# ShuhangGu/DASR

Measured on AMD Instinct MI355X. Metric: SR train images/sec (4x, 128->512), higher is better.
Workload: dtype bf16 MFMA operands, fp32 accumulate / fp32 residual stream

## Files before the change

dasr_amd/csrc/common.h:

```cpp
#pragma once
#include <hip/hip_runtime.h>
#include <hip/hip_ext.h>
#include <stdint.h>
#include "../../include/dasr_hip.h"

typedef __bf16 bf16_t;
typedef __attribute__((ext_vector_type(8))) __bf16 bf16x8;
typedef __attribute__((ext_vector_type(4))) __bf16 bf16x4;
typedef __attribute__((ext_vector_type(4))) short s16x4;
typedef _Float16 f16_t;
typedef __attribute__((ext_vector_type(8))) _Float16 f16x8;
typedef __attribute__((ext_vector_type(4))) _Float16 f16x4;
typedef __attribute__((ext_vector_type(16))) float f32x16;
typedef __attribute__((ext_vector_type(4))) float f32x4;
typedef __attribute__((ext_vector_type(4))) unsigned int u32x4;
typedef __attribute__((ext_vector_type(2))) unsigned int u32x2;

#define DASR_LDS __attribute__((address_space(3)))

#define HIP_TRY(expr)                                   \
    do {                                                \
        hipError_t _e = (expr);                         \
        if (_e != hipSuccess) return (int)_e;           \
    } while (0)

__device__ __forceinline__ float bf16_to_f32(bf16_t v) { return (float)v; }

__device__ __forceinline__ bf16_t f32_to_bf16(float v) { return (bf16_t)v; }

__device__ __forceinline__ void split_bf16(float v, bf16_t& hi, bf16_t& lo) {
    hi = (bf16_t)v;
    lo = (bf16_t)(v - (float)hi);
}

__device__ __forceinline__ void split_f16(float v, bf16_t& hi, bf16_t& lo) {
    const f16_t h = (f16_t)v;
    hi = __builtin_bit_cast(bf16_t, h);
    lo = __builtin_bit_cast(bf16_t, (f16_t)(v - (float)h));
}

template <bool F16>
__device__ __forceinline__ f32x16 mfma16(bf16x8 a, bf16x8 b, f32x16 c) {
    if constexpr (F16) return __builtin_amdgcn_mfma_f32_32x32x16_f16(__builtin_bit_cast(f16x8, a), __builtin_bit_cast(f16x8, b), c, 0, 0, 0);
    else return __builtin_amdgcn_mfma_f32_32x32x16_bf16(a, b, c, 0, 0, 0);
}

__device__ __forceinline__ float wave_sum(float v) {
#pragma unroll
    for (int o = 32; o > 0; o >>= 1) v += __shfl_xor(v, o, 64);
    return v;
}

static inline hipStream_t as_stream(void* s) { return (hipStream_t)s; }

struct dasr_red {
    float* part;
    unsigned* ticket;
};
dasr_red dasr_red_scratch(const void* key_acc, hipStream_t s, unsigned nblocks, int k);
int dasr_red_error();

template <int K>
__device__ __forceinline__ void grid_sum_commit(const dasr_red r, const float (&v)[K], float* const (&acc)[K], const float (&coef)[K]) {
    if (!r.part) return;
    __shared__ unsigned gs_last;
    __shared__ float gs_red[K][4];
    const unsigned nb = gridDim.x;
    if (threadIdx.x == 0) {
#pragma unroll
        for (int k = 0; k < K; ++k) __hip_atomic_store(r.part + (size_t)k * nb + blockIdx.x, v[k], __ATOMIC_RELAXED, __HIP_MEMORY_SCOPE_AGENT);
        asm volatile("s_waitcnt vmcnt(0)" ::: "memory");
        gs_last = __hip_atomic_fetch_add(r.ticket, 1u, __ATOMIC_RELAXED, __HIP_MEMORY_SCOPE_AGENT) == nb - 1u;
    }
    __syncthreads();
    if (!gs_last) return;
#pragma unroll
    for (int k = 0; k < K; ++k) {
        float s = 0.f;
        for (unsigned i = threadIdx.x; i < nb; i += 256u) s += __hip_atomic_load(r.part + (size_t)k * nb + i, __ATOMIC_RELAXED, __HIP_MEMORY_SCOPE_AGENT);
        s = wave_sum(s);
        if ((threadIdx.x & 63) == 0) gs_red[k][threadIdx.x >> 6] = s;
    }
    __syncthreads();
    if (threadIdx.x == 0) {
#pragma unroll
        for (int k = 0; k < K; ++k)
            if (acc[k]) atomicAdd(acc[k], ((gs_red[k][0] + gs_red[k][1]) + (gs_red[k][2] + gs_red[k][3])) * coef[k]);
        __hip_atomic_store(r.ticket, 0u, __ATOMIC_RELAXED, __HIP_MEMORY_SCOPE_AGENT);
    }
}

bool dasr_prof_slot(const char* tag, hipEvent_t* e0, hipEvent_t* e1);
#define DASR_LAUNCH_TAG(tag, kfn, grid, block, lds, s, ...)                                         \
    do {                                                                                            \
        hipEvent_t _e0 = nullptr, _e1 = nullptr;                                                    \
        if (dasr_prof_slot(tag, &_e0, &_e1)) hipExtLaunchKernelGGL(kfn, grid, block, lds, s, _e0, _e1, 0, __VA_ARGS__); \
        else hipLaunchKernelGGL(kfn, grid, block, lds, s, __VA_ARGS__);                             \
    } while (0)
#define DASR_LAUNCH(kfn, ...) DASR_LAUNCH_TAG(#kfn, kfn, __VA_ARGS__)
```

dasr_amd/csrc/misc.hip:

```cpp
#include "common.h"
#include <string.h>
#include <atomic>
#include <condition_variable>
#include <map>
#include <mutex>
#include <thread>
#include <tuple>

namespace {

__global__ void pack_kernel(const dasr_pack_desc* __restrict__ descs, int ndesc, long long total,
                            const long long* __restrict__ prefix, const float* __restrict__ params, bf16_t* __restrict__ packed) {
    const long long gid = (long long)blockIdx.x * blockDim.x + threadIdx.x;
    if (gid >= total) return;
    int lo = 0, hi = ndesc - 1;
    while (lo < hi) {
        const int mid = (lo + hi + 1) >> 1;
        if (prefix[mid] <= gid) lo = mid; else hi = mid - 1;
    }
    const dasr_pack_desc& D = descs[lo];
    long long q = gid - prefix[lo];
    const int lane = q & 63;
    q >>= 6;
    const int mi = q % D.mt;
    q /= D.mt;
    const int tap = q % D.ntaps;
    q /= D.ntaps;
    const int nchunks = D.cin_pad >> 4;
    const int ckv = q % nchunks;
    const int mg = q / nchunks;
    const int oc = (mg * D.mt + mi) * 32 + (lane & 31);
    const int kreal = D.fmt >= 3 ? nchunks / 3 : nchunks;
    const int part = ckv / kreal, ck = ckv - part * kreal;
    const int c0 = ck * 16 + 8 * (lane >> 5);
    bf16x8 vh, vl;
#pragma unroll
    for (int e = 0; e < 8; ++e) {
        const int cin = c0 + e;
        float v = 0.f;
        if (oc < D.cout) {
            for (int s = 0; s < D.nseg; ++s) {
                const dasr_pack_seg& S = D.seg[s];
                const int ci = cin - S.cin_start;
                if (ci >= 0 && ci < S.cin_len) {
                    const int st = D.tapmap[tap];
                    const unsigned msk = tap < 16 ? D.tapmask[tap] : 0u;
                    const bool okc = !S.transpose || ci < S.src_cout;
                    const long long base = !S.transpose ? S.src_off + ((long long)oc * S.src_cin + S.src_c0 + ci) * D.src_ntaps
                                                        : S.src_off + ((long long)ci * S.src_cin + S.src_c0 + oc) * D.src_ntaps;
                    if (msk && okc) {
                        float acc = 0.f;
                        for (int k = 0; k < D.src_ntaps && k < 16; ++k)
                            if (msk & (1u << k)) acc += params[base + k];
                        v = acc;
                    } else if (st >= 0 && okc) {
                        v = params[base + st];
                    }
                }
            }
        }
        bf16_t h, l;
        split_bf16(v, h, l);
        if (D.fmt == 1) h = __builtin_bit_cast(bf16_t, (f16_t)v);
        if (D.fmt == 2 || D.fmt == 3) split_f16(v, h, l);
        if (D.fmt >= 3 && part == 2) h = l;
        vh[e] = h;
        vl[e] = l;
    }
    const long long o = D.dst_off + (gid - prefix[lo]) * 8;
    *(bf16x8*)(packed + o) = vh;
    if (D.lo_off) *(bf16x8*)(packed + o + D.lo_off) = vl;
}

__global__ void nchw_to_blocked_kernel(const float* __restrict__ src, int N, int C, int H, int W, dasr_tensor df, dasr_tensor db) {
    const int ncb = (C + 15) >> 4;
    const long long total = (long long)N * ncb * H * W;
    const long long i = (long long)blockIdx.x * blockDim.x + threadIdx.x;
    if (i >= total) return;
    const int x = i % W;
    long long t = i / W;
    const int y = t % H;
    t /= H;
    const int cb = t % ncb;
    const int n = t / ncb;
    float v[16];
#pragma unroll
    for (int j = 0; j < 16; ++j) {
        const int c = cb * 16 + j;
        v[j] = c < C ? src[(((long long)n * C + c) * H + y) * W + x] : 0.f;
    }
    const size_t po = ((size_t)y * W + x) * 16;
    if (df.p) {
        float* d = (float*)df.p + (size_t)n * df.n_stride + (size_t)cb * df.cb_stride + po;
#pragma unroll
        for (int j = 0; j < 4; ++j) ((f32x4*)d)[j] = f32x4{v[4 * j], v[4 * j + 1], v[4 * j + 2], v[4 * j + 3]};
    }
    if (db.p) {
        bf16_t* d = (bf16_t*)db.p + (size_t)n * db.n_stride + (size_t)cb * db.cb_stride + po;
        bf16x8 a, b;
#pragma unroll
        for (int j = 0; j < 8; ++j) {
            a[j] = (bf16_t)v[j];
            b[j] = (bf16_t)v[8 + j];
        }
        ((bf16x8*)d)[0] = a;
        ((bf16x8*)d)[1] = b;
    }
}

__global__ void blocked_to_nchw_kernel(dasr_tensor s, int N, int C, int H, int W, float* __restrict__ dst) {
    const long long total = (long long)N * C * H * W;
    const long long i = (long long)blockIdx.x * blockDim.x + threadIdx.x;
    if (i >= total) return;
    const int x = i % W;
    long long t = i / W;
    const int y = t % H;
    t /= H;
    const int c = t % C;
    const int n = t / C;
    dst[i] = ((const float*)s.p)[(size_t)n * s.n_stride + (size_t)(c >> 4) * s.cb_stride + ((size_t)y * W + x) * 16 + (c & 15)];
}

__global__ void l1_loss_kernel(dasr_tensor sr, const float* __restrict__ hr, const float* __restrict__ wm, int N, int C, int H, int W,
                               float coef, float* loss_acc, dasr_tensor grad, int accumulate, float gscale, dasr_red rs) {
    const long long total = (long long)N * H * W;
    const long long i = (long long)blockIdx.x * blockDim.x + threadIdx.x;
    float part = 0.f;
    if (i < total) {
        const int x = i % W;
        long long t = i / W;
        const int y = t % H;
        const int n = t / H;
        const size_t po = ((size_t)y * W + x) * 16;
        const float* s = (const float*)sr.p + (size_t)n * sr.n_stride + po;
        const float wgt = wm ? wm[((long long)n * H + y) * W + x] : 1.f;
        float g[16];
#pragma unroll
        for (int j = 0; j < 16; ++j) g[j] = 0.f;
        for (int c = 0; c < C; ++c) {
            const float d = s[c] - hr[(((long long)n * C + c) * H + y) * W + x];
            if (accumulate & 2) {
                part += wgt * d * d;
                g[c] = 2.f * coef * wgt * d;
            } else {
                part += wgt * fabsf(d);
                g[c] = coef * wgt * (d > 0.f ? 1.f : (d < 0.f ? -1.f : 0.f));
            }
        }
        if (grad.p && (accumulate & 4)) {
            f16_t* gp = (f16_t*)grad.p + (size_t)n * grad.n_stride + po;
            for (int j = 0; j < (C + 3) / 4; ++j) {
                f16x4 o;
#pragma unroll
                for (int e = 0; e < 4; ++e) o[e] = (f16_t)(g[4 * j + e] * gscale);
                ((f16x4*)gp)[j] = o;
            }
        } else if (grad.p) {
            float* gp = (float*)grad.p + (size_t)n * grad.n_stride + po;
#pragma unroll
            for (int j = 0; j < 4; ++j) {
                f32x4 o = {g[4 * j], g[4 * j + 1], g[4 * j + 2], g[4 * j + 3]};
                if (accumulate & 1) o += ((const f32x4*)gp)[j];
                ((f32x4*)gp)[j] = o;
            }
        }
    }
    part = wave_sum(part);
    __shared__ float red[4];
    if ((threadIdx.x & 63) == 0) red[threadIdx.x >> 6] = part;
    __syncthreads();
    const float v[1] = {red[0] + red[1] + red[2] + red[3]};
    float* const acc[1] = {loss_acc};
    const float cf[1] = {coef};
    grid_sum_commit<1>(rs, v, acc, cf);
}

__global__ void downsum2x_kernel(dasr_tensor src, int N, int C, int H, int W, dasr_tensor mask, int mask_f32, float slope,
                                 dasr_tensor df, dasr_tensor db) {
    const int ncb = (C + 15) >> 4;
    const long long total = (long long)N * ncb * H * W * 4;
    const long long gi = (long long)blockIdx.x * blockDim.x + threadIdx.x;
    if (gi >= total) return;
    const int q = gi & 3;
    const long long i = gi >> 2;
    const int x = i % W;
    long long t = i / W;
    const int y = t % H;
    t /= H;
    const int cb = t % ncb;
    const int n = t / ncb;
    const float* s = (const float*)src.p + (size_t)n * src.n_stride + (size_t)cb * src.cb_stride + q * 4;
    const int W2 = 2 * W;
    f32x4 a = *(const f32x4*)(s + ((size_t)(2 * y) * W2 + 2 * x) * 16);
    a += *(const f32x4*)(s + ((size_t)(2 * y) * W2 + 2 * x + 1) * 16);
    a += *(const f32x4*)(s + ((size_t)(2 * y + 1) * W2 + 2 * x) * 16);
    a += *(const f32x4*)(s + ((size_t)(2 * y + 1) * W2 + 2 * x + 1) * 16);
    const size_t po = ((size_t)y * W + x) * 16 + q * 4;
    if (mask.p) {
        const size_t mo = (size_t)n * mask.n_stride + (size_t)cb * mask.cb_stride + po;
        float m[4];
        if (mask_f32) {
            const f32x4 mv = *(const f32x4*)((const float*)mask.p + mo);
            for (int j = 0; j < 4; ++j) m[j] = mv[j];
        } else {
            const bf16x4 mv = *(const bf16x4*)((const bf16_t*)mask.p + mo);
            for (int j = 0; j < 4; ++j) m[j] = (float)mv[j];
        }
        for (int j = 0; j < 4; ++j) a[j] = m[j] > 0.f ? a[j] : a[j] * slope;
    }
    if (df.p) *(f32x4*)((float*)df.p + (size_t)n * df.n_stride + (size_t)cb * df.cb_stride + po) = a;
    if (db.p) {
        bf16x4 o;
        for (int j = 0; j < 4; ++j) o[j] = (bf16_t)a[j];
        *(bf16x4*)((bf16_t*)db.p + (size_t)n * db.n_stride + (size_t)cb * db.cb_stride + po) = o;
    }
}

__global__ void axpby_kernel(dasr_tensor x, float a, dasr_tensor z, float b, int N, int C, int H, int W, dasr_tensor of,
                             dasr_tensor ob, float gamma, dasr_tensor mask, float slope, const float* slope_ptr) {
    const int ncb = (C + 15) >> 4;
    const long long per_plane = (long long)H * W * 4;
    const long long total = (long long)N * ncb * per_plane;
    const long long gi = (long long)blockIdx.x * blockDim.x + threadIdx.x;
    if (gi >= total) return;
    const long long e = (gi % per_plane) * 4;
    long long t = gi / per_plane;
    const int cb = t % ncb;
    const int n = t / ncb;
    f32x4 v = *(const f32x4*)((const float*)x.p + (size_t)n * x.n_stride + (size_t)cb * x.cb_stride + e) * a;
    if (z.p) v += *(const f32x4*)((const float*)z.p + (size_t)n * z.n_stride + (size_t)cb * z.cb_stride + e) * b;
    if (mask.p) {
        const float sl = slope_ptr ? *slope_ptr : slope;
        const f32x4 mv = *(const f32x4*)((const float*)mask.p + (size_t)n * mask.n_stride + (size_t)cb * mask.cb_stride + e);
        for (int j = 0; j < 4; ++j) v[j] = mv[j] > 0.f ? v[j] : v[j] * sl;
    }
    if (of.p) *(f32x4*)((float*)of.p + (size_t)n * of.n_stride + (size_t)cb * of.cb_stride + e) = v;
    if (ob.p) {
        bf16x4 o;
        for (int j = 0; j < 4; ++j) o[j] = (bf16_t)(v[j] * gamma);
        *(bf16x4*)((bf16_t*)ob.p + (size_t)n * ob.n_stride + (size_t)cb * ob.cb_stride + e) = o;
    }
}

__global__ void adam_kernel(float* __restrict__ p, const float* __restrict__ g, float* __restrict__ m, float* __restrict__ v,
                            long long n, float step_size, float beta1, float beta2, float eps, float wd, float inv_sqrt_bc2, int* __restrict__ nonfinite,
                            const int* __restrict__ gate) {
    if (gate && *gate != 0) return;
    bool bad = false;
    for (long long i = (long long)blockIdx.x * blockDim.x + threadIdx.x; i < n; i += (long long)gridDim.x * blockDim.x) {
        float gi = g[i];
        bad |= !(fabsf(gi) <= 3.0e38f);
        const float pi = p[i];
        if (wd != 0.f) gi += wd * pi;
        const float mi = beta1 * m[i] + (1.f - beta1) * gi;
        const float vi = beta2 * v[i] + (1.f - beta2) * gi * gi;
        m[i] = mi;
        v[i] = vi;
        const float denom = sqrtf(vi) * inv_sqrt_bc2 + eps;
        p[i] = pi - step_size * (mi / denom);
    }
    if (nonfinite && __any(bad) && (threadIdx.x & 63) == 0) atomicOr(nonfinite, 1);
}

__global__ void add_flat_kernel(float* __restrict__ y, const float* __restrict__ x, long long n) {
    for (long long i = (long long)blockIdx.x * blockDim.x + threadIdx.x; i < n; i += (long long)gridDim.x * blockDim.x) y[i] += x[i];
}

__global__ void fill_kernel(float* p, long long n, float v) {
    for (long long i = (long long)blockIdx.x * blockDim.x + threadIdx.x; i < n; i += (long long)gridDim.x * blockDim.x) p[i] = v;
}

inline unsigned blocks_for(long long total, int bs = 256) { return (unsigned)((total + bs - 1) / bs); }

}

extern "C" int dasr_pack_weights(const dasr_pack_desc* descs_dev, int32_t ndesc, int64_t total_pieces, const int64_t* piece_prefix_dev,
                                 const float* params_flat, void* packed, void* stream) {
    if (ndesc <= 0 || total_pieces <= 0) return DASR_EINVAL;
    DASR_LAUNCH(pack_kernel, dim3(blocks_for(total_pieces)), dim3(256), 0, as_stream(stream), descs_dev, ndesc,
                       (long long)total_pieces, (const long long*)piece_prefix_dev, params_flat, (bf16_t*)packed);
    return (int)hipGetLastError();
}

extern "C" int dasr_nchw_to_blocked(const float* src, int32_t N, int32_t C, int32_t H, int32_t W, dasr_tensor dst_f32,
                                    dasr_tensor dst_bf16, void* stream) {
    const long long total = (long long)N * ((C + 15) / 16) * H * W;
    if (total <= 0) return DASR_EINVAL;
    DASR_LAUNCH(nchw_to_blocked_kernel, dim3(blocks_for(total)), dim3(256), 0, as_stream(stream), src, N, C, H, W, dst_f32, dst_bf16);
    return (int)hipGetLastError();
}

extern "C" int dasr_blocked_to_nchw(dasr_tensor src, int32_t N, int32_t C, int32_t H, int32_t W, float* dst, void* stream) {
    const long long total = (long long)N * C * H * W;
    if (total <= 0) return DASR_EINVAL;
    DASR_LAUNCH(blocked_to_nchw_kernel, dim3(blocks_for(total)), dim3(256), 0, as_stream(stream), src, N, C, H, W, dst);
    return (int)hipGetLastError();
}

extern "C" int dasr_l1_loss(dasr_tensor sr, const float* hr_nchw, const float* weight_map, int32_t N, int32_t C, int32_t H, int32_t W,
                            float coef, float* loss_acc, dasr_tensor grad, int32_t accumulate, float grad_scale, void* stream) {
    const long long total = (long long)N * H * W;
    if (total <= 0 || C > 16) return DASR_EINVAL;
    if ((accumulate & 4) && (accumulate & 1)) return DASR_EINVAL;
    const dasr_red rs = dasr_red_scratch(loss_acc, as_stream(stream), blocks_for(total), 1);
    if (loss_acc && !rs.part) return dasr_red_error();
    DASR_LAUNCH(l1_loss_kernel, dim3(blocks_for(total)), dim3(256), 0, as_stream(stream), sr, hr_nchw, weight_map, N, C, H, W, coef,
                       loss_acc, grad, accumulate, grad_scale != 0.f ? grad_scale : 1.f, rs);
    return (int)hipGetLastError();
}

extern "C" int dasr_downsum2x(dasr_tensor src, int32_t N, int32_t C, int32_t H, int32_t W, dasr_tensor mask, int32_t mask_f32,
                              float slope, dasr_tensor dst_f32, dasr_tensor dst_bf16, void* stream) {
    const long long total = (long long)N * ((C + 15) / 16) * H * W * 4;
    if (total <= 0) return DASR_EINVAL;
    DASR_LAUNCH(downsum2x_kernel, dim3(blocks_for(total)), dim3(256), 0, as_stream(stream), src, N, C, H, W, mask, mask_f32, slope,
                       dst_f32, dst_bf16);
    return (int)hipGetLastError();
}

__device__ __forceinline__ float f32_rounded(float v) {
    asm("" : "+v"(v));
    return v;
}

__global__ void cvt_f16_kernel(dasr_tensor x, int N, int C, int H, int W, float scale, dasr_tensor y) {
    const int ncb = (C + 15) >> 4;
    const long long per_plane = (long long)H * W * 4, total = (long long)N * ncb * per_plane;
    const long long gi = (long long)blockIdx.x * blockDim.x + threadIdx.x;
    if (gi >= total) return;
    const long long e = (gi % per_plane) * 4;
    long long t = gi / per_plane;
    const int cb = t % ncb, n = t / ncb;
    const f32x4 v = *(const f32x4*)((const float*)x.p + (size_t)n * x.n_stride + (size_t)cb * x.cb_stride + e);
    f16x4 o;
    for (int j = 0; j < 4; ++j) o[j] = (f16_t)f32_rounded(v[j] * scale);
    *(f16x4*)((f16_t*)y.p + (size_t)n * y.n_stride + (size_t)cb * y.cb_stride + e) = o;
}

__global__ void f16_residual_kernel(dasr_tensor x, int N, int C, int H, int W, float scale, dasr_tensor y) {
    const int ncb = (C + 15) >> 4;
    const long long per_plane = (long long)H * W * 4, total = (long long)N * ncb * per_plane;
    const long long gi = (long long)blockIdx.x * blockDim.x + threadIdx.x;
    if (gi >= total) return;
    const long long e = (gi % per_plane) * 4;
    long long t = gi / per_plane;
    const int cb = t % ncb, n = t / ncb;
    const f32x4 v = *(const f32x4*)((const float*)x.p + (size_t)n * x.n_stride + (size_t)cb * x.cb_stride + e);
    const float inv = 1.f / scale;
    f32x4 o;
    for (int j = 0; j < 4; ++j) o[j] = v[j] - (float)(f16_t)f32_rounded(v[j] * scale) * inv;
    *(f32x4*)((float*)y.p + (size_t)n * y.n_stride + (size_t)cb * y.cb_stride + e) = o;
}

template <typename T>
__global__ void cvt_split16_kernel(dasr_tensor x, int N, int C, int H, int W, float scale, dasr_tensor y) {
    const int ncb = (C + 15) >> 4;
    const long long per_plane = (long long)H * W * 4, total = (long long)N * ncb * per_plane;
    const long long gi = (long long)blockIdx.x * blockDim.x + threadIdx.x;
    if (gi >= total) return;
    const long long e = (gi % per_plane) * 4;
    long long t = gi / per_plane;
    const int cb = t % ncb, n = t / ncb;
    const f32x4 v = *(const f32x4*)((const float*)x.p + (size_t)n * x.n_stride + (size_t)cb * x.cb_stride + e);
    T* yp = (T*)y.p + (size_t)n * y.n_stride + (size_t)cb * y.cb_stride + e;
    const size_t lo = (size_t)ncb * y.cb_stride;
#pragma unroll
    for (int j = 0; j < 4; ++j) {
        const float vv = f32_rounded(v[j] * scale);
        const T h = (T)vv;
        yp[j] = h;
        yp[lo + j] = (T)(vv - (float)h);
    }
}

__global__ void downsum2x_f16_kernel(dasr_tensor src, int N, int C, int H, int W, dasr_tensor mask, float slope, float out_scale, dasr_tensor df,
                                     dasr_tensor dh) {
    const int ncb = (C + 15) >> 4;
    const long long total = (long long)N * ncb * H * W * 4;
    const long long gi = (long long)blockIdx.x * blockDim.x + threadIdx.x;
    if (gi >= total) return;
    const int q = gi & 3;
    const long long i = gi >> 2;
    const int x = i % W;
    long long t = i / W;
    const int y = t % H;
    t /= H;
    const int cb = t % ncb, n = t / ncb;
    const f16_t* s = (const f16_t*)src.p + (size_t)n * src.n_stride + (size_t)cb * src.cb_stride + q * 4;
    const int W2 = 2 * W;
    float a[4] = {0.f, 0.f, 0.f, 0.f};
    for (int dy = 0; dy < 2; ++dy)
        for (int dx = 0; dx < 2; ++dx) {
            const f16x4 v = *(const f16x4*)(s + ((size_t)(2 * y + dy) * W2 + 2 * x + dx) * 16);
            for (int j = 0; j < 4; ++j) a[j] += (float)v[j];
        }
    const size_t po = ((size_t)y * W + x) * 16 + q * 4;
    if (mask.p) {
        const f16x4 mv = *(const f16x4*)((const f16_t*)mask.p + (size_t)n * mask.n_stride + (size_t)cb * mask.cb_stride + po);
        for (int j = 0; j < 4; ++j) a[j] = (float)mv[j] > 0.f ? a[j] : a[j] * slope;
    }
    for (int j = 0; j < 4; ++j) a[j] *= out_scale;
    if (df.p) *(f32x4*)((float*)df.p + (size_t)n * df.n_stride + (size_t)cb * df.cb_stride + po) = f32x4{a[0], a[1], a[2], a[3]};
    if (dh.p) {
        f16x4 o;
        for (int j = 0; j < 4; ++j) o[j] = (f16_t)a[j];
        *(f16x4*)((f16_t*)dh.p + (size_t)n * dh.n_stride + (size_t)cb * dh.cb_stride + po) = o;
    }
}

__global__ void pixel_shuffle_f16_kernel(dasr_tensor src, int N, int C4, int H, int W, dasr_tensor dst) {
    const int ncb = C4 >> 4;
    const long long total = (long long)N * ncb * H * W;
    const long long i = (long long)blockIdx.x * blockDim.x + threadIdx.x;
    if (i >= total) return;
    const int x = i % W;
    long long t = i / W;
    const int y = t % H;
    t /= H;
    const int p = t % ncb, n = t / ncb;
    const f16_t* s = (const f16_t*)src.p + (size_t)n * src.n_stride + (size_t)p * src.cb_stride + ((size_t)y * W + x) * 16;
    const f16x8 lo = *(const f16x8*)s, hi = *(const f16x8*)(s + 8);
    f16_t v[16];
    for (int j = 0; j < 8; ++j) { v[j] = lo[j]; v[8 + j] = hi[j]; }
    f16_t* d = (f16_t*)dst.p + (size_t)n * dst.n_stride + (size_t)(p >> 2) * dst.cb_stride + 4 * (p & 3);
    const int W2 = 2 * W;
    for (int k = 0; k < 4; ++k) {
        const f16x4 o = {v[k], v[4 + k], v[8 + k], v[12 + k]};
        *(f16x4*)(d + ((size_t)(2 * y + (k >> 1)) * W2 + 2 * x + (k & 1)) * 16) = o;
    }
}

__global__ void pixel_unshuffle_f16_kernel(dasr_tensor gsrc, dasr_tensor mask, float slope, int N, int C4, int H, int W, dasr_tensor gdst) {
    const int ncb = C4 >> 4;
    const long long total = (long long)N * ncb * H * W;
    const long long i = (long long)blockIdx.x * blockDim.x + threadIdx.x;
    if (i >= total) return;
    const int x = i % W;
    long long t = i / W;
    const int y = t % H;
    t /= H;
    const int p = t % ncb, n = t / ncb;
    const f16_t* g = (const f16_t*)gsrc.p + (size_t)n * gsrc.n_stride + (size_t)(p >> 2) * gsrc.cb_stride + 4 * (p & 3);
    const int W2 = 2 * W;
    f16_t v[16];
    for (int k = 0; k < 4; ++k) {
        const f16x4 q = *(const f16x4*)(g + ((size_t)(2 * y + (k >> 1)) * W2 + 2 * x + (k & 1)) * 16);
        for (int cc = 0; cc < 4; ++cc) v[4 * cc + k] = q[cc];
    }
    const size_t po = (size_t)n * gdst.n_stride + (size_t)p * gdst.cb_stride + ((size_t)y * W + x) * 16;
    if (mask.p) {
        const f16_t* m = (const f16_t*)mask.p + (size_t)n * mask.n_stride + (size_t)p * mask.cb_stride + ((size_t)y * W + x) * 16;
        for (int j = 0; j < 16; ++j) v[j] = (float)m[j] > 0.f ? v[j] : (f16_t)((float)v[j] * slope);
    }
    f16x8 lo, hi;
    for (int j = 0; j < 8; ++j) { lo[j] = v[j]; hi[j] = v[8 + j]; }
    *(f16x8*)((f16_t*)gdst.p + po) = lo;
    *(f16x8*)((f16_t*)gdst.p + po + 8) = hi;
}

extern "C" int dasr_pixel_shuffle_f16(dasr_tensor src, int32_t N, int32_t C4, int32_t H, int32_t W, dasr_tensor dst, void* stream) {
    const long long total = (long long)N * (C4 / 16) * H * W;
    if (total <= 0 || (C4 & 63) || !src.p || !dst.p) return DASR_EINVAL;
    DASR_LAUNCH(pixel_shuffle_f16_kernel, dim3(blocks_for(total)), dim3(256), 0, as_stream(stream), src, N, C4, H, W, dst);
    return (int)hipGetLastError();
}

extern "C" int dasr_pixel_unshuffle_f16(dasr_tensor gsrc, dasr_tensor mask, float slope, int32_t N, int32_t C4, int32_t H, int32_t W, dasr_tensor gdst,
                                        void* stream) {
    const long long total = (long long)N * (C4 / 16) * H * W;
    if (total <= 0 || (C4 & 63) || !gsrc.p || !gdst.p) return DASR_EINVAL;
    DASR_LAUNCH(pixel_unshuffle_f16_kernel, dim3(blocks_for(total)), dim3(256), 0, as_stream(stream), gsrc, mask, slope, N, C4, H, W, gdst);
    return (int)hipGetLastError();
}

extern "C" int dasr_cvt_f16(dasr_tensor x, int32_t N, int32_t C, int32_t H, int32_t W, float scale, dasr_tensor y, void* stream) {
    const long long total = (long long)N * ((C + 15) / 16) * H * W * 4;
    if (total <= 0 || !x.p || !y.p) return DASR_EINVAL;
    DASR_LAUNCH(cvt_f16_kernel, dim3(blocks_for(total)), dim3(256), 0, as_stream(stream), x, N, C, H, W, scale, y);
    return (int)hipGetLastError();
}

extern "C" int dasr_cvt_split16(dasr_tensor x, int32_t N, int32_t C, int32_t H, int32_t W, float scale, dasr_tensor y, int32_t f16, void* stream) {
    const long long total = (long long)N * ((C + 15) / 16) * H * W * 4;
    if (total <= 0 || !x.p || !y.p) return DASR_EINVAL;
    if (f16) DASR_LAUNCH(cvt_split16_kernel<f16_t>, dim3(blocks_for(total)), dim3(256), 0, as_stream(stream), x, N, C, H, W, scale, y);
    else DASR_LAUNCH(cvt_split16_kernel<bf16_t>, dim3(blocks_for(total)), dim3(256), 0, as_stream(stream), x, N, C, H, W, scale, y);
    return (int)hipGetLastError();
}

extern "C" int dasr_f16_residual(dasr_tensor x, int32_t N, int32_t C, int32_t H, int32_t W, float scale, dasr_tensor y, void* stream) {
    const long long total = (long long)N * ((C + 15) / 16) * H * W * 4;
    if (total <= 0 || !x.p || !y.p || !(scale > 0.f)) return DASR_EINVAL;
    DASR_LAUNCH(f16_residual_kernel, dim3(blocks_for(total)), dim3(256), 0, as_stream(stream), x, N, C, H, W, scale, y);
    return (int)hipGetLastError();
}

extern "C" int dasr_downsum2x_f16(dasr_tensor src, int32_t N, int32_t C, int32_t H, int32_t W, dasr_tensor mask, float slope, float out_scale,
                                  dasr_tensor dst_f32, dasr_tensor dst_f16, void* stream) {
    const long long total = (long long)N * ((C + 15) / 16) * H * W * 4;
    if (total <= 0 || !src.p) return DASR_EINVAL;
    DASR_LAUNCH(downsum2x_f16_kernel, dim3(blocks_for(total)), dim3(256), 0, as_stream(stream), src, N, C, H, W, mask, slope, out_scale, dst_f32, dst_f16);
    return (int)hipGetLastError();
}

extern "C" int dasr_axpby(dasr_tensor x, float a, dasr_tensor z, float b, int32_t N, int32_t C, int32_t H, int32_t W,
                          dasr_tensor out_f32, dasr_tensor out_bf16, float gamma, dasr_tensor mask, float slope, const float* slope_ptr,
                          void* stream) {
    const long long total = (long long)N * ((C + 15) / 16) * H * W * 4;
    if (total <= 0) return DASR_EINVAL;
    DASR_LAUNCH(axpby_kernel, dim3(blocks_for(total)), dim3(256), 0, as_stream(stream), x, a, z, b, N, C, H, W, out_f32, out_bf16, gamma, mask, slope, slope_ptr);
    return (int)hipGetLastError();
}

extern "C" int dasr_adam(float* p, const float* g, float* m, float* v, int64_t n, float lr, float beta1, float beta2, float eps,
                         float weight_decay, int32_t step, int32_t* nonfinite_flag, const int32_t* gate_flag, void* stream) {
    if (n <= 0 || step <= 0) return DASR_EINVAL;
    const double bc1 = 1.0 - pow((double)beta1, (double)step), bc2 = 1.0 - pow((double)beta2, (double)step);
    const float step_size = (float)((double)lr / bc1);
    const float inv_sqrt_bc2 = (float)(1.0 / sqrt(bc2));
    const unsigned blocks = (unsigned)((n + 255) / 256 < 4096 ? (n + 255) / 256 : 4096);
    DASR_LAUNCH(adam_kernel, dim3(blocks), dim3(256), 0, as_stream(stream), p, g, m, v, (long long)n, step_size, beta1, beta2, eps,
                       weight_decay, inv_sqrt_bc2, nonfinite_flag, gate_flag);
    return (int)hipGetLastError();
}

extern "C" int dasr_fill_f32(float* p, int64_t n, float value, void* stream) {
    if (n <= 0) return DASR_EINVAL;
    const unsigned blocks = (unsigned)((n + 255) / 256 < 4096 ? (n + 255) / 256 : 4096);
    DASR_LAUNCH(fill_kernel, dim3(blocks), dim3(256), 0, as_stream(stream), p, (long long)n, value);
    return (int)hipGetLastError();
}

extern "C" int dasr_add_flat(float* y, const float* x, int64_t n, void* stream) {
    if (n <= 0) return DASR_EINVAL;
    const unsigned blocks = (unsigned)((n + 255) / 256 < 4096 ? (n + 255) / 256 : 4096);
    DASR_LAUNCH(add_flat_kernel, dim3(blocks), dim3(256), 0, as_stream(stream), y, x, (long long)n);
    return (int)hipGetLastError();
}

__global__ void gather_crops_kernel(const dasr_crop_desc* __restrict__ descs, int n, int C, int size, float* __restrict__ dst) {
    const long long total = (long long)n * C * size * size;
    const long long i = (long long)blockIdx.x * blockDim.x + threadIdx.x;
    if (i >= total) return;
    const int x = i % size;
    long long t = i / size;
    const int y = t % size;
    t /= size;
    const int c = t % C;
    const int k = t / C;
    const dasr_crop_desc D = descs[k];
    int ci = y, cj = x;
    if (D.flags & 4) { ci = x; cj = y; }
    if (D.flags & 2) ci = size - 1 - ci;
    if (D.flags & 1) cj = size - 1 - cj;
    const int vy = D.y0 + ci, vx = D.x0 + cj;
    float v = 0.f;
    if (c < D.C && vy >= 0 && vy < D.vH && vx >= 0 && vx < D.vW) {
        const float* s = D.src + (size_t)c * D.H * D.W;
        if (D.vH == D.H && D.vW == D.W) {
            v = s[(size_t)vy * D.W + vx];
        } else {
            float fy = ((float)vy + 0.5f) * ((float)D.H / (float)D.vH) - 0.5f, fx = ((float)vx + 0.5f) * ((float)D.W / (float)D.vW) - 0.5f;
            int y0 = (int)floorf(fy), x0 = (int)floorf(fx);
            const float wy = fy - (float)y0, wx = fx - (float)x0;
            const int y1 = min(max(y0 + 1, 0), D.H - 1), x1 = min(max(x0 + 1, 0), D.W - 1);
            y0 = min(max(y0, 0), D.H - 1);
            x0 = min(max(x0, 0), D.W - 1);
            v = (1.f - wy) * ((1.f - wx) * s[(size_t)y0 * D.W + x0] + wx * s[(size_t)y0 * D.W + x1]) +
                wy * ((1.f - wx) * s[(size_t)y1 * D.W + x0] + wx * s[(size_t)y1 * D.W + x1]);
        }
    }
    dst[i] = v;
}

extern "C" int dasr_gather_crops(const dasr_crop_desc* descs_dev, int32_t n, int32_t C, int32_t size, float* dst, void* stream) {
    const long long total = (long long)n * C * size * size;
    if (total <= 0 || !descs_dev || !dst) return DASR_EINVAL;
    DASR_LAUNCH(gather_crops_kernel, dim3((unsigned)((total + 255) / 256)), dim3(256), 0, as_stream(stream), descs_dev, n, C, size, dst);
    return (int)hipGetLastError();
}

extern "C" void* dasr_event_create(void) {
    hipEvent_t e = nullptr;
    if (hipEventCreateWithFlags(&e, hipEventDisableTiming) != hipSuccess) return nullptr;
    return (void*)e;
}

extern "C" int dasr_event_destroy(void* ev) { return ev ? (int)hipEventDestroy((hipEvent_t)ev) : 0; }

extern "C" int dasr_abi_version(void) { return DASR_ABI_VERSION; }

static thread_local int g_last_failed_op = -1;
extern "C" int dasr_last_failed_op(void) { return g_last_failed_op; }

namespace {
struct RedRow {
    char* base;
    size_t floats;
};
std::mutex g_red_mu;
std::map<std::tuple<int, const void*, hipStream_t>, RedRow> g_red_rows;
thread_local bool g_red_capture_refused = false;
}

int dasr_red_error() {
    const bool c = g_red_capture_refused;
    g_red_capture_refused = false;
    return c ? DASR_ECAPTURE : DASR_EINVAL;
}

// ... 324 lines not shown
```

Baseline: 554.6.

## Stage weight-pack source rows in LDS and batch L1 loss pixel groups

The weight pack kernel now gives each block a quantum of pieces, resolves per-cin source rows once, and stages the source rows into LDS. Taps and output pieces are then emitted from shared memory instead of each thread gathering strided params. This cuts redundant global gathers. The L1 loss kernel is templated to process several 256-pixel groups per block with vector loads when C<=4. It keeps per-group partial sums so the grid reduction stays the same, and grid_sum is split into a commit and finish step to allow this. The cost is more code complexity and extra block syncs in the pack kernel.

```diff
diff --git a/dasr_amd/csrc/common.h b/dasr_amd/csrc/common.h
--- a/dasr_amd/csrc/common.h
+++ b/dasr_amd/csrc/common.h
@@ -61,23 +61,19 @@
 int dasr_red_error();
 
 template <int K>
-__device__ __forceinline__ void grid_sum_commit(const dasr_red r, const float (&v)[K], float* const (&acc)[K], const float (&coef)[K]) {
-    if (!r.part) return;
+__device__ __forceinline__ void grid_sum_finish(const dasr_red r, const unsigned np, float* const (&acc)[K], const float (&coef)[K]) {
     __shared__ unsigned gs_last;
     __shared__ float gs_red[K][4];
-    const unsigned nb = gridDim.x;
     if (threadIdx.x == 0) {
-#pragma unroll
-        for (int k = 0; k < K; ++k) __hip_atomic_store(r.part + (size_t)k * nb + blockIdx.x, v[k], __ATOMIC_RELAXED, __HIP_MEMORY_SCOPE_AGENT);
         asm volatile("s_waitcnt vmcnt(0)" ::: "memory");
-        gs_last = __hip_atomic_fetch_add(r.ticket, 1u, __ATOMIC_RELAXED, __HIP_MEMORY_SCOPE_AGENT) == nb - 1u;
+        gs_last = __hip_atomic_fetch_add(r.ticket, 1u, __ATOMIC_RELAXED, __HIP_MEMORY_SCOPE_AGENT) == gridDim.x - 1u;
     }
     __syncthreads();
     if (!gs_last) return;
 #pragma unroll
     for (int k = 0; k < K; ++k) {
         float s = 0.f;
-        for (unsigned i = threadIdx.x; i < nb; i += 256u) s += __hip_atomic_load(r.part + (size_t)k * nb + i, __ATOMIC_RELAXED, __HIP_MEMORY_SCOPE_AGENT);
+        for (unsigned i = threadIdx.x; i < np; i += 256u) s += __hip_atomic_load(r.part + (size_t)k * np + i, __ATOMIC_RELAXED, __HIP_MEMORY_SCOPE_AGENT);
         s = wave_sum(s);
         if ((threadIdx.x & 63) == 0) gs_red[k][threadIdx.x >> 6] = s;
     }
@@ -90,6 +86,16 @@
     }
 }
 
+template <int K>
+__device__ __forceinline__ void grid_sum_commit(const dasr_red r, const float (&v)[K], float* const (&acc)[K], const float (&coef)[K]) {
+    if (!r.part) return;
+    if (threadIdx.x == 0) {
+#pragma unroll
+        for (int k = 0; k < K; ++k) __hip_atomic_store(r.part + (size_t)k * gridDim.x + blockIdx.x, v[k], __ATOMIC_RELAXED, __HIP_MEMORY_SCOPE_AGENT);
+    }
+    grid_sum_finish<K>(r, gridDim.x, acc, coef);
+}
+
 bool dasr_prof_slot(const char* tag, hipEvent_t* e0, hipEvent_t* e1);
 #define DASR_LAUNCH_TAG(tag, kfn, grid, block, lds, s, ...)                                         \
     do {                                                                                            \
diff --git a/dasr_amd/csrc/misc.hip b/dasr_amd/csrc/misc.hip
--- a/dasr_amd/csrc/misc.hip
+++ b/dasr_amd/csrc/misc.hip
@@ -9,67 +9,118 @@
 
 namespace {
 
-__global__ void pack_kernel(const dasr_pack_desc* __restrict__ descs, int ndesc, long long total,
-                            const long long* __restrict__ prefix, const float* __restrict__ params, bf16_t* __restrict__ packed) {
-    const long long gid = (long long)blockIdx.x * blockDim.x + threadIdx.x;
-    if (gid >= total) return;
+constexpr int PACK_Q = 2048;
+constexpr int PACK_NT_LDS = 16;
+__host__ __device__ constexpr int pack_cin_stride(int nt) { return 32 * nt + (33 * nt) % 64; }
+constexpr int PACK_LDS = 16 * pack_cin_stride(PACK_NT_LDS);
+
+__global__ __launch_bounds__(256) void pack_kernel(const dasr_pack_desc* __restrict__ descs, int ndesc, long long total, int quantum,
+                                                   const long long* __restrict__ prefix, const float* __restrict__ params, bf16_t* __restrict__ packed) {
+    __shared__ float src[PACK_LDS];
+    __shared__ long long rowbase[16];
+    __shared__ int rowstride[16];
+    __shared__ int rowtr[16];
+    const int tid = threadIdx.x, lane = tid & 63, wave = __builtin_amdgcn_readfirstlane(tid >> 6);
+    const long long q0 = (long long)blockIdx.x * quantum, q1 = q0 + quantum < total ? q0 + quantum : total;
     int lo = 0, hi = ndesc - 1;
     while (lo < hi) {
         const int mid = (lo + hi + 1) >> 1;
-        if (prefix[mid] <= gid) lo = mid; else hi = mid - 1;
-    }
-    const dasr_pack_desc& D = descs[lo];
-    long long q = gid - prefix[lo];
-    const int lane = q & 63;
-    q >>= 6;
-    const int mi = q % D.mt;
-    q /= D.mt;
-    const int tap = q % D.ntaps;
-    q /= D.ntaps;
-    const int nchunks = D.cin_pad >> 4;
-    const int ckv = q % nchunks;
-    const int mg = q / nchunks;
-    const int oc = (mg * D.mt + mi) * 32 + (lane & 31);
-    const int kreal = D.fmt >= 3 ? nchunks / 3 : nchunks;
-    const int part = ckv / kreal, ck = ckv - part * kreal;
-    const int c0 = ck * 16 + 8 * (lane >> 5);
-    bf16x8 vh, vl;
-#pragma unroll
-    for (int e = 0; e < 8; ++e) {
-        const int cin = c0 + e;
-        float v = 0.f;
-        if (oc < D.cout) {
-            for (int s = 0; s < D.nseg; ++s) {
-                const dasr_pack_seg& S = D.seg[s];
-                const int ci = cin - S.cin_start;
-                if (ci >= 0 && ci < S.cin_len) {
-                    const int st = D.tapmap[tap];
-                    const unsigned msk = tap < 16 ? D.tapmask[tap] : 0u;
-                    const bool okc = !S.transpose || ci < S.src_cout;
-                    const long long base = !S.transpose ? S.src_off + ((long long)oc * S.src_cin + S.src_c0 + ci) * D.src_ntaps
-                                                        : S.src_off + ((long long)ci * S.src_cin + S.src_c0 + oc) * D.src_ntaps;
-                    if (msk && okc) {
-                        float acc = 0.f;
-                        for (int k = 0; k < D.src_ntaps && k < 16; ++k)
-                            if (msk & (1u << k)) acc += params[base + k];
-                        v = acc;
-                    } else if (st >= 0 && okc) {
-                        v = params[base + st];
+        if (prefix[mid] <= q0) lo = mid; else hi = mid - 1;
+    }
+    for (int d = lo; d < ndesc; ++d) {
+        const long long p0 = prefix[d];
+        if (p0 >= q1) break;
+        const dasr_pack_desc& D = descs[d];
+        const int ntaps = D.ntaps, mt = D.mt, nt = D.src_ntaps, fmt = D.fmt, cout = D.cout;
+        const int tp = ntaps * mt * 64;
+        if (tp <= 0) continue;
+        const int ntile = (int)((prefix[d + 1] - p0) / tp);
+        const int nchunks = D.cin_pad >> 4;
+        const int kreal = fmt >= 3 ? nchunks / 3 : nchunks;
+        const bool staged = nt <= PACK_NT_LDS;
+        const int cs = pack_cin_stride(nt);
+        for (int t = p0 >= q0 ? 0 : (int)((q0 - p0 + tp - 1) / tp); t < ntile && p0 + (long long)t * tp < q1; ++t) {
+            const int mg = t / nchunks, ckv = t - mg * nchunks;
+            const int part = ckv / kreal, ck = ckv - part * kreal;
+            if (tid < 16) {
+                const int cin = ck * 16 + tid;
+                long long base = -1;
+                int stride = 0, tr = 0;
+                for (int s = 0; s < D.nseg; ++s) {
+                    const dasr_pack_seg& S = D.seg[s];
+                    const int ci = cin - S.cin_start;
+                    if (ci < 0 || ci >= S.cin_len || (S.transpose && ci >= S.src_cout)) continue;
+                    tr = S.transpose != 0;
+                    base = !tr ? S.src_off + (long long)(S.src_c0 + ci) * nt : S.src_off + ((long long)ci * S.src_cin + S.src_c0) * nt;
+                    stride = !tr ? S.src_cin * nt : nt;
+                }
+                rowbase[tid] = base;
+                rowstride[tid] = stride;
+                rowtr[tid] = tr;
+            }
+            __syncthreads();
+            for (int mi = 0; mi < mt; ++mi) {
+                const int oc0 = (mg * mt + mi) * 32;
+                const int nrows = cout - oc0 < 0 ? 0 : (cout - oc0 < 32 ? cout - oc0 : 32);
+                if (staged) {
+                    for (int c = wave; c < 16; c += 4) {
+                        if (!rowtr[c]) continue;
+                        const long long b = rowbase[c];
+                        const float* g = params + (b < 0 ? 0 : b + (long long)oc0 * nt);
+                        const int n = b < 0 ? 0 : nrows * nt;
+                        for (int j = lane; j < 32 * nt; j += 64) src[c * cs + j] = j < n ? g[j] : 0.f;
                     }
+                    for (int e = lane; e < 16 * nt; e += 64) {
+                        const int c = e / nt, k = e - c * nt;
+                        if (rowtr[c]) continue;
+                        const long long b = rowbase[c];
+                        const int st = rowstride[c];
+                        float* dst = src + c * cs + k;
+#pragma unroll
+                        for (int i = 0; i < 8; ++i) {
+                            const int r = wave + 4 * i;
+                            dst[r * nt] = (b >= 0 && r < nrows) ? params[b + (long long)(oc0 + r) * st + k] : 0.f;
+                        }
+                    }
+                    __syncthreads();
                 }
+                const int r = lane & 31, c0 = 8 * (lane >> 5);
+                auto emit = [&](auto row_of) {
+                    for (int tap = wave; tap < ntaps; tap += 4) {
+                        const int st = D.tapmap[tap];
+                        const unsigned msk = tap < 16 ? D.tapmask[tap] : 0u;
+                        bf16x8 vh, vl;
+#pragma unroll
+                        for (int e = 0; e < 8; ++e) {
+                            const auto row = row_of(c0 + e);
+                            float v = 0.f;
+                            if (row && msk) {
+                                float acc = 0.f;
+                                for (int k = 0; k < nt && k < 16; ++k)
+                                    if (msk & (1u << k)) acc += row[k];
+                                v = acc;
+                            } else if (row && st >= 0) {
+                                v = row[st];
+                            }
+                            bf16_t h, l;
+                            split_bf16(v, h, l);
+                            if (fmt == 1) h = __builtin_bit_cast(bf16_t, (f16_t)v);
+                            if (fmt == 2 || fmt == 3) split_f16(v, h, l);
+                            if (fmt >= 3 && part == 2) h = l;
+                            vh[e] = h;
+                            vl[e] = l;
+                        }
+                        const long long o = D.dst_off + ((long long)t * tp + ((tap * mt + mi) * 64 + lane)) * 8;
+                        *(bf16x8*)(packed + o) = vh;
+                        if (D.lo_off) *(bf16x8*)(packed + o + D.lo_off) = vl;
+                    }
+                };
+                if (staged) emit([&](int c) { return &src[c * cs + r * nt]; });
+                else emit([&](int c) { return (rowbase[c] >= 0 && r < nrows) ? params + rowbase[c] + (long long)(oc0 + r) * rowstride[c] : (const float*)nullptr; });
+                __syncthreads();
             }
         }
-        bf16_t h, l;
-        split_bf16(v, h, l);
-        if (D.fmt == 1) h = __builtin_bit_cast(bf16_t, (f16_t)v);
-        if (D.fmt == 2 || D.fmt == 3) split_f16(v, h, l);
-        if (D.fmt >= 3 && part == 2) h = l;
-        vh[e] = h;
-        vl[e] = l;
-    }
-    const long long o = D.dst_off + (gid - prefix[lo]) * 8;
-    *(bf16x8*)(packed + o) = vh;
-    if (D.lo_off) *(bf16x8*)(packed + o + D.lo_off) = vl;
+    }
 }
 
 __global__ void nchw_to_blocked_kernel(const float* __restrict__ src, int N, int C, int H, int W, dasr_tensor df, dasr_tensor db) {
@@ -121,58 +172,101 @@
     dst[i] = ((const float*)s.p)[(size_t)n * s.n_stride + (size_t)(c >> 4) * s.cb_stride + ((size_t)y * W + x) * 16 + (c & 15)];
 }
 
-__global__ void l1_loss_kernel(dasr_tensor sr, const float* __restrict__ hr, const float* __restrict__ wm, int N, int C, int H, int W,
-                               float coef, float* loss_acc, dasr_tensor grad, int accumulate, float gscale, dasr_red rs) {
-    const long long total = (long long)N * H * W;
-    const long long i = (long long)blockIdx.x * blockDim.x + threadIdx.x;
-    float part = 0.f;
-    if (i < total) {
-        const int x = i % W;
-        long long t = i / W;
-        const int y = t % H;
-        const int n = t / H;
-        const size_t po = ((size_t)y * W + x) * 16;
-        const float* s = (const float*)sr.p + (size_t)n * sr.n_stride + po;
-        const float wgt = wm ? wm[((long long)n * H + y) * W + x] : 1.f;
-        float g[16];
-#pragma unroll
-        for (int j = 0; j < 16; ++j) g[j] = 0.f;
-        for (int c = 0; c < C; ++c) {
-            const float d = s[c] - hr[(((long long)n * C + c) * H + y) * W + x];
+template <int NV, int G>
+__global__ __launch_bounds__(256) void l1_loss_kernel(dasr_tensor sr, const float* __restrict__ hr, const float* __restrict__ wm, int N, int C, int H, int W,
+                                                      float coef, float* loss_acc, dasr_tensor grad, int accumulate, float gscale, dasr_red rs, unsigned ngroups) {
+#pragma clang fp contract(off)
+    const long long HW = (long long)H * W, total = (long long)N * HW;
+    const int tid = threadIdx.x;
+    bool live[G];
+    size_t so[G];
+    int img[G];
+    f32x4 s4[G][NV];
+    float h[G][4 * NV], wgt[G];
+#pragma unroll
+    for (int q = 0; q < G; ++q) {
+        const long long base = ((long long)blockIdx.x * G + q) * 256;
+        long long n = base / HW, p = base - n * HW + tid;
+        while (p >= HW) {
+            p -= HW;
+            ++n;
+        }
+        live[q] = base + tid < total;
+        img[q] = (int)n;
+        so[q] = (size_t)p * 16;
+        wgt[q] = 1.f;
+#pragma unroll
+        for (int j = 0; j < NV; ++j) s4[q][j] = f32x4{0.f, 0.f, 0.f, 0.f};
+#pragma unroll
+        for (int c = 0; c < 4 * NV; ++c) h[q][c] = 0.f;
+        if (live[q]) {
+            const f32x4* s = (const f32x4*)((const float*)sr.p + (size_t)n * sr.n_stride + so[q]);
+#pragma unroll
+            for (int j = 0; j < NV; ++j) s4[q][j] = s[j];
+#pragma unroll
+            for (int c = 0; c < 4 * NV; ++c)
+                if (c < C) h[q][c] = hr[(n * C + c) * HW + p];
+            if (wm) wgt[q] = wm[n * HW + p];
+        }
+    }
+    float part[G];
+#pragma unroll
+    for (int q = 0; q < G; ++q) {
+        part[q] = 0.f;
+        if (!live[q]) continue;
+        float g[4 * NV];
+#pragma unroll
+        for (int c = 0; c < 4 * NV; ++c) {
+            g[c] = 0.f;
+            if (c >= C) continue;
+            const float d = s4[q][c >> 2][c & 3] - h[q][c];
             if (accumulate & 2) {
-                part += wgt * d * d;
-                g[c] = 2.f * coef * wgt * d;
+                part[q] += wgt[q] * d * d;
+                g[c] = 2.f * coef * wgt[q] * d;
             } else {
-                part += wgt * fabsf(d);
-                g[c] = coef * wgt * (d > 0.f ? 1.f : (d < 0.f ? -1.f : 0.f));
+                part[q] += wgt[q] * fabsf(d);
+                g[c] = coef * wgt[q] * (d > 0.f ? 1.f : (d < 0.f ? -1.f : 0.f));
             }
         }
         if (grad.p && (accumulate & 4)) {
-            f16_t* gp = (f16_t*)grad.p + (size_t)n * grad.n_stride + po;
-            for (int j = 0; j < (C + 3) / 4; ++j) {
+            f16_t* gp = (f16_t*)grad.p + (size_t)img[q] * grad.n_stride + so[q];
+#pragma unroll
+            for (int j = 0; j < NV; ++j) {
+                if (j >= (C + 3) / 4) break;
                 f16x4 o;
 #pragma unroll
                 for (int e = 0; e < 4; ++e) o[e] = (f16_t)(g[4 * j + e] * gscale);
                 ((f16x4*)gp)[j] = o;
             }
         } else if (grad.p) {
-            float* gp = (float*)grad.p + (size_t)n * grad.n_stride + po;
+            float* gp = (float*)grad.p + (size_t)img[q] * grad.n_stride + so[q];
 #pragma unroll
             for (int j = 0; j < 4; ++j) {
-                f32x4 o = {g[4 * j], g[4 * j + 1], g[4 * j + 2], g[4 * j + 3]};
+                f32x4 o = {0.f, 0.f, 0.f, 0.f};
+                if (j < NV) o = f32x4{g[4 * j], g[4 * j + 1], g[4 * j + 2], g[4 * j + 3]};
                 if (accumulate & 1) o += ((const f32x4*)gp)[j];
                 ((f32x4*)gp)[j] = o;
             }
         }
     }
-    part = wave_sum(part);
-    __shared__ float red[4];
-    if ((threadIdx.x & 63) == 0) red[threadIdx.x >> 6] = part;
+    if (!rs.part) return;
+    __shared__ float red[G][4];
+#pragma unroll
+    for (int q = 0; q < G; ++q) {
+        const float w = wave_sum(part[q]);
+        if ((tid & 63) == 0) red[q][tid >> 6] = w;
+    }
     __syncthreads();
-    const float v[1] = {red[0] + red[1] + red[2] + red[3]};
+    if (tid == 0) {
+#pragma unroll
+        for (int q = 0; q < G; ++q) {
+            const unsigned b = blockIdx.x * G + q;
+            if (b < ngroups) __hip_atomic_store(rs.part + b, red[q][0] + red[q][1] + red[q][2] + red[q][3], __ATOMIC_RELAXED, __HIP_MEMORY_SCOPE_AGENT);
+        }
+    }
     float* const acc[1] = {loss_acc};
     const float cf[1] = {coef};
-    grid_sum_commit<1>(rs, v, acc, cf);
+    grid_sum_finish<1>(rs, ngroups, acc, cf);
 }
 
 __global__ void downsum2x_kernel(dasr_tensor src, int N, int C, int H, int W, dasr_tensor mask, int mask_f32, float slope,
@@ -277,8 +371,10 @@
 extern "C" int dasr_pack_weights(const dasr_pack_desc* descs_dev, int32_t ndesc, int64_t total_pieces, const int64_t* piece_prefix_dev,
                                  const float* params_flat, void* packed, void* stream) {
     if (ndesc <= 0 || total_pieces <= 0) return DASR_EINVAL;
-    DASR_LAUNCH(pack_kernel, dim3(blocks_for(total_pieces)), dim3(256), 0, as_stream(stream), descs_dev, ndesc,
-                       (long long)total_pieces, (const long long*)piece_prefix_dev, params_flat, (bf16_t*)packed);
+    long long quantum = (total_pieces / 2048 + 63) / 64 * 64;
+    quantum = quantum < 64 ? 64 : (quantum > PACK_Q ? PACK_Q : quantum);
+    DASR_LAUNCH(pack_kernel, dim3(blocks_for(total_pieces, (int)quantum)), dim3(256), 0, as_stream(stream), descs_dev, ndesc,
+                       (long long)total_pieces, (int)quantum, (const long long*)piece_prefix_dev, params_flat, (bf16_t*)packed);
     return (int)hipGetLastError();
 }
 
@@ -302,10 +398,12 @@
     const long long total = (long long)N * H * W;
     if (total <= 0 || C > 16) return DASR_EINVAL;
     if ((accumulate & 4) && (accumulate & 1)) return DASR_EINVAL;
-    const dasr_red rs = dasr_red_scratch(loss_acc, as_stream(stream), blocks_for(total), 1);
+    const unsigned ngroups = blocks_for(total);
+    const dasr_red rs = dasr_red_scratch(loss_acc, as_stream(stream), ngroups, 1);
     if (loss_acc && !rs.part) return dasr_red_error();
-    DASR_LAUNCH(l1_loss_kernel, dim3(blocks_for(total)), dim3(256), 0, as_stream(stream), sr, hr_nchw, weight_map, N, C, H, W, coef,
-                       loss_acc, grad, accumulate, grad_scale != 0.f ? grad_scale : 1.f, rs);
+    const float gs = grad_scale != 0.f ? grad_scale : 1.f;
+    if (C <= 4) DASR_LAUNCH((l1_loss_kernel<1, 4>), dim3((ngroups + 3) / 4), dim3(256), 0, as_stream(stream), sr, hr_nchw, weight_map, N, C, H, W, coef, loss_acc, grad, accumulate, gs, rs, ngroups);
+    else DASR_LAUNCH((l1_loss_kernel<4, 1>), dim3(ngroups), dim3(256), 0, as_stream(stream), sr, hr_nchw, weight_map, N, C, H, W, coef, loss_acc, grad, accumulate, gs, rs, ngroups);
     return (int)hipGetLastError();
 }
 
```

Result: faster. 560.3 (median of 6 runs) (+1.0%).
